# kjedrzejewski/video-cycle_gan-upscaling

Measured on AMD Instinct MI355X. Metric: upscaled frames/s (train step, G+D fwd+bwd) at 256->512, higher is better.
Workload: dtype f32; 1 GPU; C2: make_upscaler_orig((512,512,3),k=3,x2,res=9) + PatchGAN-70, batch 8/GPU, gan2 wiring, Wasserstein + pixel-MSE, faithful 3-call step incl. predict pass; global_batch=8, frame=256x256->512x512, parallelism=dp1, launch=hipGraph replay

## Files before the change

### video-cycle_gan-upscaling_amd/build.py

```python
import glob
import os
import subprocess
import sys
from concurrent.futures import ThreadPoolExecutor

HERE = os.path.dirname(os.path.abspath(__file__))
ROOT = os.path.dirname(HERE)
CSRC = os.path.join(HERE, "csrc")
OUT = os.path.join(HERE, "libvcg_hip.so")
SOURCES = ["conv_fwd.hip", "conv_rowchain.hip", "conv_transpose.hip", "conv_wgrad.hip", "norm.hip", "elementwise.hip", "dense.hip", "bf16_layout.hip", "bf16_conv3x3_3ch.hip", "bf16_convt3x3.hip", "bf16_conv9x9_to3.hip", "bf16_norm.hip", "bf16_wgrad.hip", "bf16_wgrad9.hip", "bf16_gconv.hip", "bf16_gwgrad.hip", "bf16_head.hip", "bf16_wgrad3.hip", "bf16_attn.hip", "bf16_incep.hip", "bf16_vgg.hip", "api.hip"]
FLAGS = ["-O3", "--offload-arch=gfx950", "-fPIC", "-std=c++17", "-I", os.path.join(ROOT, "include"), "-I", CSRC,
         "-Wno-unused-value", "-Wno-c++20-extensions"]


def _hipcc():
    for c in (os.environ.get("HIPCC"), "/opt/rocm/bin/hipcc", "hipcc"):
        if c and (os.path.isabs(c) and os.path.exists(c) or not os.path.isabs(c)):
            return c
    raise RuntimeError("hipcc not found")


def _stale(target, deps):
    if not os.path.exists(target):
        return True
    t = os.path.getmtime(target)
    return any(os.path.getmtime(d) > t for d in deps)


def build(force=False, verbose=True, extra_flags=(), objdir=None, out=OUT, jobs=4):
    hipcc = _hipcc()
    objdir = objdir or os.path.join(HERE, "build")
    flags = FLAGS + list(extra_flags)
    hdrs = sorted(glob.glob(os.path.join(CSRC, "*.hpp"))) + [os.path.join(ROOT, "include", "vcg.h")]
    objs, cmds = [], []
    os.makedirs(objdir, exist_ok=True)
    for s in SOURCES:
        src = os.path.join(CSRC, s)
        obj = os.path.join(objdir, s.replace(".hip", ".o"))
        objs.append(obj)
        if force or _stale(obj, [src] + hdrs):
            cmds.append([hipcc, "-c", src, "-o", obj] + flags)

    def run(cmd):
        if verbose:
            print(" ".join(cmd), flush=True)
        subprocess.run(cmd, check=True)

    with ThreadPoolExecutor(max_workers=jobs) as ex:
        list(ex.map(run, cmds))
    if force or cmds or _stale(out, objs):
        run([hipcc, "-shared", "-fPIC", "--offload-arch=gfx950", "-o", out] + objs)
    return out


if __name__ == "__main__":
    print(build(force="--force" in sys.argv))
```

### video-cycle_gan-upscaling_amd/csrc/api.hip

```cpp
#include "vcg_common.hpp"

int vcg_internal_conv(const float* x, const float* w, float* y, int n, int cin, int h, int wd, int cout, int oh,
                      int ow, int kh, int kw, int stride, int pad_top, int pad_left, int flip, const vcg_epilogue* ep,
                      int smallm, int ws_t, int ws_m, int ws_k, hipStream_t st, float* stats = nullptr, const float* scale = nullptr,
                      const float* shift = nullptr);
int vcg_internal_convt(const float* x, const float* w, float* y, int n, int cin, int h, int wd, int cout, int oh,
                       int ow, int k, int cby, int cbx, const vcg_epilogue* ep, hipStream_t st);
size_t vcg_internal_wgrad_ws(int n, int mtot, int ah, int aw, int jctot, int kh, int kw, int S);
int vcg_internal_wgrad(const float* A, const float* B, float* dw, float* db, int n, int mtot, int ah, int aw,
                       int jctot, int bh, int bw, int kh, int kw, int S, int pt, int pl_, int flip, int ts, int sm,
                       int sj, void* ws, size_t ws_bytes, hipStream_t st);

namespace {

int check_desc(const vcg_conv_desc* d) {
    if (d == nullptr) return VCG_E_NULL;
    if (d->n <= 0 || d->cin <= 0 || d->h <= 0 || d->w <= 0 || d->cout <= 0 || d->oh <= 0 || d->ow <= 0)
        return VCG_E_SHAPE;
    if (d->kh <= 0 || d->kw <= 0 || d->stride < 1 || d->stride > 3) return VCG_E_UNSUPPORTED;
    if (d->pad_top < 0 || d->pad_left < 0 || d->pad_top >= d->kh || d->pad_left >= d->kw) return VCG_E_SHAPE;
    return VCG_OK;
}

inline bool use_smallm(int mch, int kh, int kw, int stride) { return stride == 1 && kh == kw && kh >= 3 && mch * kw <= 32; }

}

extern "C" {

const char* vcg_version(void) { return "vcg-hip 0.1 (gfx950, fp32 MFMA 32x32x2)"; }

const char* vcg_error_string(int code) {
    switch (code) {
        case VCG_OK: return "ok";
        case VCG_E_NULL: return "required pointer is NULL";
        case VCG_E_SHAPE: return "inconsistent or unsupported dimensions";
        case VCG_E_UNSUPPORTED: return "kernel size / stride / padding combination not instantiated";
        case VCG_E_WORKSPACE: return "workspace missing or too small";
        default: return code > 0 ? hipGetErrorString((hipError_t)code) : "unknown error";
    }
}

int vcg_conv2d_fwd(const vcg_conv_desc* d, const float* x, const float* w_hwio, float* y, const vcg_epilogue* ep,
                   vcg_stream_t stream) {
    int rc = check_desc(d);
    if (rc) return rc;
    VCG_CHECK_PTR(x); VCG_CHECK_PTR(w_hwio); VCG_CHECK_PTR(y);
    if ((d->oh - 1) * d->stride - d->pad_top >= d->h || (d->ow - 1) * d->stride - d->pad_left >= d->w) return VCG_E_SHAPE;
    const bool sm = use_smallm(d->cout, d->kh, d->kw, d->stride);
    return vcg_internal_conv(x, w_hwio, y, d->n, d->cin, d->h, d->w, d->cout, d->oh, d->ow, d->kh, d->kw, d->stride,
                             d->pad_top, d->pad_left, 0, ep, sm ? 1 : 0, d->cin * d->cout, 1, d->cout,
                             (hipStream_t)stream);
}

static bool conv_stats_tiles(const vcg_conv_desc* d, int* tiles_per_image) {
    const bool k3 = d->kh == 3 && d->kw == 3, k4 = d->kh == 4 && d->kw == 4;
    if (!(k3 || k4) || d->stride > 2 || d->cin <= 3) return false;
    const bool sm = use_smallm(d->cout, d->kh, d->kw, d->stride);
    if (sm) return false;
    const int xt = (k3 && d->stride == 1 && d->ow > 32) ? 2 : 1;
    *tiles_per_image = ceil_div(d->ow, 32 * xt) * ceil_div(d->oh, 8);
    return true;
}

int vcg_conv2d_stats_records(const vcg_conv_desc* d, int stats_mode) {
    int rc = check_desc(d);
    if (rc) return rc;
    int tpi = 0;
    if (!conv_stats_tiles(d, &tpi) || (stats_mode != VCG_STATS_BATCH && stats_mode != VCG_STATS_INSTANCE)) return VCG_E_UNSUPPORTED;
    const long all = (long)tpi * d->n;
    if (all > 0x3fffffffL) return VCG_E_UNSUPPORTED;
    return (int)(stats_mode == VCG_STATS_INSTANCE ? tpi : all);
}

int vcg_conv2d_fwd_stats(const vcg_conv_desc* d, const float* x, const float* w_hwio, const float* bias, float* y, float* stats,
                         vcg_stream_t stream) {
    int rc = check_desc(d);
    if (rc) return rc;
    VCG_CHECK_PTR(x); VCG_CHECK_PTR(w_hwio); VCG_CHECK_PTR(y); VCG_CHECK_PTR(stats);
    if ((d->oh - 1) * d->stride - d->pad_top >= d->h || (d->ow - 1) * d->stride - d->pad_left >= d->w) return VCG_E_SHAPE;
    int tpi = 0;
    if (!conv_stats_tiles(d, &tpi)) return VCG_E_UNSUPPORTED;
    vcg_epilogue ep{};
    ep.bias = bias;
    ep.act = VCG_ACT_NONE;
    return vcg_internal_conv(x, w_hwio, y, d->n, d->cin, d->h, d->w, d->cout, d->oh, d->ow, d->kh, d->kw, d->stride, d->pad_top, d->pad_left, 0,
                             &ep, 0, d->cin * d->cout, 1, d->cout, (hipStream_t)stream, stats);
}

int vcg_conv2d_fwd_affine(const vcg_conv_desc* d, const float* x, const float* w_hwio, float* y, const vcg_epilogue* ep, const float* scale,
                          const float* shift, vcg_stream_t stream) {
    int rc = check_desc(d);
    if (rc) return rc;
    VCG_CHECK_PTR(x); VCG_CHECK_PTR(w_hwio); VCG_CHECK_PTR(y); VCG_CHECK_PTR(scale); VCG_CHECK_PTR(shift);
    if ((d->oh - 1) * d->stride - d->pad_top >= d->h || (d->ow - 1) * d->stride - d->pad_left >= d->w) return VCG_E_SHAPE;
    if (use_smallm(d->cout, d->kh, d->kw, d->stride)) return VCG_E_UNSUPPORTED;
    return vcg_internal_conv(x, w_hwio, y, d->n, d->cin, d->h, d->w, d->cout, d->oh, d->ow, d->kh, d->kw, d->stride, d->pad_top, d->pad_left, 0,
                             ep, 0, d->cin * d->cout, 1, d->cout, (hipStream_t)stream, nullptr, scale, shift);
}

int vcg_conv2d_dgrad(const vcg_conv_desc* d, const float* dy, const float* w_hwio, const float* w_hwoi, float* dx,
                     const float* residual, vcg_stream_t stream) {
    int rc = check_desc(d);
    if (rc) return rc;
    VCG_CHECK_PTR(dy); VCG_CHECK_PTR(dx);
    vcg_epilogue ep{};
    ep.residual = residual;
    hipStream_t st = (hipStream_t)stream;
    if (d->stride == 1) {
        const int pt = d->kh - 1 - d->pad_top, pl = d->kw - 1 - d->pad_left;
        if (use_smallm(d->cin, d->kh, d->kw, 1)) {
            VCG_CHECK_PTR(w_hwio);
            return vcg_internal_conv(dy, w_hwio, dx, d->n, d->cout, d->oh, d->ow, d->cin, d->h, d->w, d->kh, d->kw, 1,
                                     pt, pl, 1, &ep, 1, d->cin * d->cout, d->cout, 1, st);
        }
        VCG_CHECK_PTR(w_hwoi);
        return vcg_internal_conv(dy, w_hwoi, dx, d->n, d->cout, d->oh, d->ow, d->cin, d->h, d->w, d->kh, d->kw, 1, pt,
                                 pl, 1, &ep, 0, 0, 0, 0, st);
    }
    if (d->kh != d->kw || d->stride != 2) return VCG_E_UNSUPPORTED;
    VCG_CHECK_PTR(w_hwoi);
    return vcg_internal_convt(dy, w_hwoi, dx, d->n, d->cout, d->oh, d->ow, d->cin, d->h, d->w, d->kh, d->pad_top,
                              d->pad_left, &ep, st);
}

size_t vcg_conv2d_wgrad_workspace_bytes(const vcg_conv_desc* d) {
    if (check_desc(d)) return 0;
    size_t a;
    if (d->stride == 1 && d->cout <= 3)
        a = vcg_internal_wgrad_ws(d->n, d->cin, d->h, d->w, d->cout, d->kh, d->kw, 1);
    else
        a = vcg_internal_wgrad_ws(d->n, d->cout, d->oh, d->ow, d->cin, d->kh, d->kw, d->stride);
    const size_t b = vcg_channel_sum_workspace_bytes(d->n, d->cout, d->oh * d->ow);
    return a > b ? a : b;
}

int vcg_conv2d_wgrad(const vcg_conv_desc* d, const float* x, const float* dy, float* dw_hwio, float* dbias, void* ws,
                     size_t ws_bytes, vcg_stream_t stream) {
    int rc = check_desc(d);
    if (rc) return rc;
    VCG_CHECK_PTR(x); VCG_CHECK_PTR(dy); VCG_CHECK_PTR(dw_hwio);
    hipStream_t st = (hipStream_t)stream;
    const int cc = d->cin * d->cout;
    if (d->stride == 1 && d->cout <= 3) {
        rc = vcg_internal_wgrad(x, dy, dw_hwio, nullptr, d->n, d->cin, d->h, d->w, d->cout, d->oh, d->ow, d->kh, d->kw,
                                1, d->kh - 1 - d->pad_top, d->kw - 1 - d->pad_left, 1, cc, d->cout, 1, ws, ws_bytes, st);
    } else {
        rc = vcg_internal_wgrad(dy, x, dw_hwio, dbias, d->n, d->cout, d->oh, d->ow, d->cin, d->h, d->w, d->kh, d->kw,
                                d->stride, d->pad_top, d->pad_left, 0, cc, 1, d->cout, ws, ws_bytes, st);
        dbias = nullptr;
    }
    if (rc) return rc;
    if (dbias) {
        if (ws_bytes < vcg_channel_sum_workspace_bytes(d->n, d->cout, d->oh * d->ow)) return VCG_E_WORKSPACE;
        rc = vcg_channel_sum(dy, d->n, d->cout, d->oh * d->ow, dbias, ws, ws_bytes, stream);
    }
    return rc;
}

int vcg_conv_transpose2d_fwd(const vcg_conv_desc* d, const float* x, const float* w_hwio_t, float* y,
                             const vcg_epilogue* ep, vcg_stream_t stream) {
    int rc = check_desc(d);
    if (rc) return rc;
    VCG_CHECK_PTR(x); VCG_CHECK_PTR(w_hwio_t); VCG_CHECK_PTR(y);
    if (d->stride != 2 || d->kh != d->kw) return VCG_E_UNSUPPORTED;
    if (d->oh > 2 * d->h || d->ow > 2 * d->w) return VCG_E_SHAPE;
    return vcg_internal_convt(x, w_hwio_t, y, d->n, d->cin, d->h, d->w, d->cout, d->oh, d->ow, d->kh, d->pad_top,
                              d->pad_left, ep, (hipStream_t)stream);
}

int vcg_conv_transpose2d_dgrad(const vcg_conv_desc* d, const float* dy, const float* w_hwoi, float* dx,
                               const float* residual, vcg_stream_t stream) {
    int rc = check_desc(d);
    if (rc) return rc;
    VCG_CHECK_PTR(dy); VCG_CHECK_PTR(w_hwoi); VCG_CHECK_PTR(dx);
    if (d->stride != 2) return VCG_E_UNSUPPORTED;
    vcg_epilogue ep{};
    ep.residual = residual;
    return vcg_internal_conv(dy, w_hwoi, dx, d->n, d->cout, d->oh, d->ow, d->cin, d->h, d->w, d->kh, d->kw, 2,
                             d->pad_top, d->pad_left, 0, &ep, 0, 0, 0, 0, (hipStream_t)stream);
}

size_t vcg_conv_transpose2d_wgrad_workspace_bytes(const vcg_conv_desc* d) {
    if (check_desc(d)) return 0;
    size_t a = vcg_internal_wgrad_ws(d->n, d->cin, d->h, d->w, d->cout, d->kh, d->kw, 2);
    size_t b = vcg_channel_sum_workspace_bytes(d->n, d->cout, d->oh * d->ow);
    return a > b ? a : b;
}

int vcg_conv_transpose2d_wgrad(const vcg_conv_desc* d, const float* x, const float* dy, float* dw_hwoi, float* dbias,
                               void* ws, size_t ws_bytes, vcg_stream_t stream) {
    int rc = check_desc(d);
    if (rc) return rc;
    VCG_CHECK_PTR(x); VCG_CHECK_PTR(dy); VCG_CHECK_PTR(dw_hwoi);
    if (d->stride != 2) return VCG_E_UNSUPPORTED;
    rc = vcg_internal_wgrad(x, dy, dw_hwoi, nullptr, d->n, d->cin, d->h, d->w, d->cout, d->oh, d->ow, d->kh, d->kw, 2,
                            d->pad_top, d->pad_left, 0, d->cin * d->cout, 1, d->cin, ws, ws_bytes, (hipStream_t)stream);
    if (rc) return rc;
    if (dbias) {
        if (ws_bytes < vcg_channel_sum_workspace_bytes(d->n, d->cout, d->oh * d->ow)) return VCG_E_WORKSPACE;
        rc = vcg_channel_sum(dy, d->n, d->cout, d->oh * d->ow, dbias, ws, ws_bytes, stream);
    }
    return rc;
}
// ... 3 lines not shown
```

### video-cycle_gan-upscaling_amd/csrc/conv_fwd.hip

```cpp
#include "vcg_common.hpp"
#include <type_traits>

namespace {

struct ConvParams {
    const float* x;
    const float* w;
    float* y;
    const float* bias;
    const float* prelu;
    const float* residual;
    int n, cin, h, w_, cout, oh, ow, pad_top, pad_left;
    int tiles_x, tiles_y, co_blocks;
    int act;
    float alpha;
    int flip;
    int ws_t, ws_m, ws_k;
    float* stats;
    const float* scale;
    const float* shift;
};

template <int KH, int KW, int S, int CK, int XT>
struct ConvCfg {
// ... 495 lines not shown
            const int ch = ci0 + ci;
            const bool ok = e < C::W_ELEMS && ch < p.cin && mi < mrows;
            const int mch = mi / KW, kx = mi % KW;
            int tap = ky * KW + kx;
            if (p.flip) tap = KH * KW - 1 - tap;
            rw[i] = buf_load(rwt, ok ? 4u * (unsigned)(tap * p.ws_t + mch * p.ws_m + ch * p.ws_k) : VCG_OOB);
        }
    };
    auto store_chunk = [&]() {
#pragma unroll
        for (int i = 0; i < C::IN_PT; ++i) {
            const int e = tid + i * 256;
            if (e < C::IN_ELEMS) s_in[e] = rin[i];
        }
#pragma unroll
        for (int i = 0; i < C::W_PT; ++i) {
            const int e = tid + i * 256;
            if (e < C::W_ELEMS) s_w[e] = rw[i];
        }
    };

    f32x16 acc[2][2];
#pragma unroll
    for (int i = 0; i < 2; ++i)
#pragma unroll
        for (int j = 0; j < 2; ++j)
#pragma unroll
            for (int r = 0; r < 16; ++r) acc[i][j][r] = 0.f;

    const float* bbase = s_in + half * C::PLANE + (wv * 2) * C::XW + l31;
    const float* abase = s_w + half * KH * 32 + l31;

    const int nchunks = (p.cin + CK - 1) / CK;
    load_chunk(0);
    for (int c = 0; c < nchunks; ++c) {
        __syncthreads();
        store_chunk();
        __syncthreads();
        if (c + 1 < nchunks) load_chunk((c + 1) * CK);
#pragma unroll
        for (int cp = 0; cp < CK / 2; ++cp) {
#pragma unroll
            for (int ky = 0; ky < KH; ++ky) {
                const float a = abase[(cp * 2 * KH + ky) * 32];
                const float b00 = bbase[cp * 2 * C::PLANE + ky * C::XW];
                const float b01 = bbase[cp * 2 * C::PLANE + ky * C::XW + 32];
                const float b10 = bbase[cp * 2 * C::PLANE + (ky + 1) * C::XW];
                const float b11 = bbase[cp * 2 * C::PLANE + (ky + 1) * C::XW + 32];
                acc[0][0] = mfma32(a, b00, acc[0][0]);
                acc[0][1] = mfma32(a, b01, acc[0][1]);
                acc[1][0] = mfma32(a, b10, acc[1][0]);
                acc[1][1] = mfma32(a, b11, acc[1][1]);
            }
        }
    }

    float* s_p = smem + wv * 32 * C::PST;
#pragma unroll
    for (int rt = 0; rt < 2; ++rt) {
        __syncthreads();
#pragma unroll
        for (int xt = 0; xt < 2; ++xt)
#pragma unroll
            for (int r = 0; r < 16; ++r) s_p[mfma_row(r, lane) * C::PST + xt * 32 + l31] = acc[rt][xt][r];
        __syncthreads();
        const int oy = oy0 + wv * 2 + rt;
        const int ox = ox0 + lane;
        if (lane < C::OUTW && oy < p.oh && ox < p.ow) {
            for (int mch = 0; mch < p.cout; ++mch) {
                float v = 0.f;
#pragma unroll
                for (int kx = 0; kx < KW; ++kx) v += s_p[(mch * KW + kx) * C::PST + lane + kx];
                const float bv = p.bias ? p.bias[mch] : 0.f;
                const float al = (p.act == VCG_ACT_PRELU) ? p.prelu[mch] : p.alpha;
                const size_t idx = (((size_t)n * p.cout + mch) * p.oh + oy) * p.ow + ox;
                v = apply_act(v + bv, p.act, al);
                if (p.residual) v += p.residual[idx];
                p.y[idx] = v;
            }
        }
    }
}

template <int K>
__global__ __launch_bounds__(256) void conv_cout1_kernel(const ConvParams p) {
    __shared__ float red[4][64];
    const int tid = threadIdx.x, xl = tid & 63;
    const int cg = __builtin_amdgcn_readfirstlane(tid >> 6);
    int b = blockIdx.x;
    const int seg = b % p.tiles_x; b /= p.tiles_x;
    const int oy = b % p.oh;
    const int n = b / p.oh;
    const int ox = seg * 64 + xl, gx0 = ox - p.pad_left, gy0 = oy - p.pad_top;
    const int hw = p.h * p.w_;
    const vcg_rsrc rx = make_rsrc(p.x + (size_t)n * p.cin * hw, (size_t)p.cin * hw * sizeof(float));
    unsigned coff[K];
#pragma unroll
    for (int kx = 0; kx < K; ++kx) coff[kx] = (unsigned)(gx0 + kx) < (unsigned)p.w_ ? 4u * (unsigned)(gx0 + kx) : VCG_OOB;
    float acc = 0.f;
#pragma unroll 1
    for (int c = cg; c < p.cin; c += 4) {
        float wr[K * K];
#pragma unroll
        for (int t = 0; t < K * K; ++t) wr[t] = p.w[(p.flip ? K * K - 1 - t : t) * p.ws_t + c * p.ws_k];
#pragma unroll
        for (int ky = 0; ky < K; ++ky) {
            const int gy = gy0 + ky;
            const bool rok = (unsigned)gy < (unsigned)p.h;
            const unsigned rbase = 4u * (unsigned)(c * hw + gy * p.w_);
#pragma unroll
            for (int kx = 0; kx < K; ++kx) acc += buf_load(rx, rok && coff[kx] != VCG_OOB ? rbase + coff[kx] : VCG_OOB) * wr[ky * K + kx];
        }
    }
    red[cg][xl] = acc;
    __syncthreads();
    if (cg == 0 && ox < p.ow) {
        float v = ((red[0][xl] + red[1][xl]) + (red[2][xl] + red[3][xl])) + (p.bias ? p.bias[0] : 0.f);
        if (p.act == VCG_ACT_LRELU) v = v >= 0.f ? v : v * p.alpha;
        else if (p.act == VCG_ACT_TANH) v = tanhf(v);
        const size_t o = ((size_t)n * p.oh + oy) * p.ow + ox;
        if (p.residual) v += p.residual[o];
        p.y[o] = v;
    }
}

template <int K>
int launch_cout1(ConvParams p, hipStream_t st) {
    p.tiles_x = ceil_div(p.ow, 64);
    const long grid = (long)p.tiles_x * p.oh * p.n;
    if (grid <= 0 || grid > 0x7fffffffL) return VCG_E_SHAPE;
    hipLaunchKernelGGL(conv_cout1_kernel<K>, dim3((unsigned)grid), dim3(256), 0, st, p);
    VCG_LAUNCH_CHECK();
    return VCG_OK;
}

template <typename Kern>
int launch_with_lds(Kern kern, int grid, size_t lds, const ConvParams& p, hipStream_t st) {
    if (int e = vcg_allow_dyn_lds(reinterpret_cast<const void*>(kern), lds)) return e;
    hipLaunchKernelGGL(kern, dim3(grid), dim3(256), lds, st, p);
    VCG_LAUNCH_CHECK();
    return VCG_OK;
}

bool conv_block_fits(int oh, int ow, int ck, int h, int w) {
    const unsigned long long lim = 0xFFFFFFE0ull;
    return 64ull * oh * ow * sizeof(float) < lim && (unsigned long long)ck * h * w * sizeof(float) < lim;
}

template <int KH, int KW, int S, int CK, int XT>
int launch_conv(ConvParams p, hipStream_t st) {
    using C = ConvCfg<KH, KW, S, CK, XT>;
    if (!conv_block_fits(p.oh, p.ow, CK, p.h, p.w_)) return VCG_E_UNSUPPORTED;
    p.tiles_x = ceil_div(p.ow, 32 * XT);
    p.tiles_y = ceil_div(p.oh, C::ROWS);
    p.co_blocks = ceil_div(p.cout, 64);
    const long grid = (long)p.tiles_x * p.tiles_y * p.co_blocks * p.n;
    if (grid <= 0 || grid > 0x7fffffffL) return VCG_E_SHAPE;
    if (p.stats && p.scale) return VCG_E_UNSUPPORTED;
    if (p.stats) {
        if constexpr ((KH == 3 && KW == 3 && S <= 2) || (KH == 4 && KW == 4 && S <= 2))
            return launch_with_lds(conv_fwd_kernel<KH, KW, S, CK, XT, true>, (int)grid, C::LDS_BYTES, p, st);
        else
            return VCG_E_UNSUPPORTED;
    }
    if (p.scale) {
        if constexpr (S == 1 && ((KH == 3 && KW == 3) || (KH == 5 && KW == 5)))
            return launch_with_lds(conv_fwd_kernel<KH, KW, S, CK, XT, false, true>, (int)grid, C::LDS_BYTES, p, st);
        else
            return VCG_E_UNSUPPORTED;
    }
    return launch_with_lds(conv_fwd_kernel<KH, KW, S, CK, XT>, (int)grid, C::LDS_BYTES, p, st);
}

int device_cu_count() {
    static const int cus = [] {
        int dev = 0, v = 0;
        if (hipGetDevice(&dev) != hipSuccess || hipDeviceGetAttribute(&v, hipDeviceAttributeMultiprocessorCount, dev) != hipSuccess) return 0;
        return v;
    }();
    return cus;
}

template <int KH, int KW, int S>
int launch_c3(ConvParams p, hipStream_t st) {
    using C = C3Cfg<KH, KW, S>;
    if (!conv_block_fits(p.oh, p.ow, 3, p.h, p.w_)) return VCG_E_UNSUPPORTED;
    p.tiles_x = ceil_div(p.ow, 32);
    p.tiles_y = ceil_div(p.oh, C::ROWS);
    p.co_blocks = ceil_div(p.cout, 64);
    const long tiles = (long)p.tiles_x * p.tiles_y * p.co_blocks * p.n;
    if (tiles <= 0 || tiles > 0x7fffffffL) return VCG_E_SHAPE;
    const int cus = device_cu_count();
    if (cus <= 0) return VCG_E_UNSUPPORTED;
    long grid = tiles < 2L * cus ? tiles : 2L * cus;
    grid -= grid % p.co_blocks;
    if (grid < p.co_blocks) grid = p.co_blocks;
    return launch_with_lds(conv_c3_kernel<KH, KW, S>, (int)grid, C::LDS_BYTES, p, st);
}

template <int KH, int KW, int CK>
int launch_smallm(ConvParams p, hipStream_t st) {
    using C = SmallCfg<KH, KW, CK>;
    p.tiles_x = ceil_div(p.ow, C::OUTW);
    p.tiles_y = ceil_div(p.oh, C::ROWS);
    p.co_blocks = 1;
    const long grid = (long)p.tiles_x * p.tiles_y * p.n;
    if (grid <= 0 || grid > 0x7fffffffL) return VCG_E_SHAPE;
    return launch_with_lds(conv_smallm_kernel<KH, KW, CK>, (int)grid, C::LDS_BYTES, p, st);
}

}

int vcg_internal_conv9_rowchain(const float* x, const float* w, float* y, int n, int cin, int h, int wd, int cout, const float* bias, int act,
                                int ws_t, int ws_m, int ws_k, hipStream_t st);

int vcg_internal_conv(const float* x, const float* w, float* y, int n, int cin, int h, int wd, int cout,
                      int oh, int ow, int kh, int kw, int stride, int pad_top, int pad_left, int flip,
                      const vcg_epilogue* ep, int smallm, int ws_t, int ws_m, int ws_k, hipStream_t st, float* stats, const float* scale, const float* shift) {
    ConvParams p{};
    p.x = x; p.w = w; p.y = y; p.stats = stats;
    if (stats && (smallm || cin <= 3)) return VCG_E_UNSUPPORTED;
    if (scale && (smallm || stats || cin <= 3)) return VCG_E_UNSUPPORTED;
    if (scale && shift == nullptr) return VCG_E_NULL;
    p.scale = scale; p.shift = scale ? shift : nullptr;
    p.bias = ep ? ep->bias : nullptr;
    p.prelu = ep ? ep->prelu_alpha : nullptr;
    p.residual = ep ? ep->residual : nullptr;
    p.act = ep ? ep->act : VCG_ACT_NONE;
    p.alpha = ep ? ep->act_alpha : 0.f;
    if (p.act == VCG_ACT_PRELU && p.prelu == nullptr) return VCG_E_NULL;
    p.n = n; p.cin = cin; p.h = h; p.w_ = wd; p.cout = cout; p.oh = oh; p.ow = ow;
    p.pad_top = pad_top; p.pad_left = pad_left; p.flip = flip;
    p.ws_t = ws_t; p.ws_m = ws_m; p.ws_k = ws_k;
    if (n <= 0 || cin <= 0 || cout <= 0 || oh <= 0 || ow <= 0) return VCG_E_SHAPE;
    if (smallm) {
        if (stride != 1 || cout * kw > 32) return VCG_E_UNSUPPORTED;
        if (kh == 9 && kw == 9 && !flip && pad_top == 4 && pad_left == 4 && oh == h && ow == wd && !p.prelu && !p.residual) {
            const int rc = vcg_internal_conv9_rowchain(x, w, y, n, cin, h, wd, cout, p.bias, p.act, ws_t, ws_m, ws_k, st);
            if (rc != VCG_E_UNSUPPORTED) return rc;
        }
        if (cout == 1 && cin >= 64 && kh == kw && ws_m == 1 && !p.prelu && (size_t)cin * h * wd * 4 <= 0xFFFFFFE0u) {
            if (kh == 3) return launch_cout1<3>(p, st);
            if (kh == 4) return launch_cout1<4>(p, st);
            if (kh == 5) return launch_cout1<5>(p, st);
        }
        if (kh == 9 && kw == 9) return launch_smallm<9, 9, 8>(p, st);
        if (kh == 4 && kw == 4) return launch_smallm<4, 4, 8>(p, st);
        if (kh == 3 && kw == 3) return launch_smallm<3, 3, 8>(p, st);
        if (kh == 5 && kw == 5) return launch_smallm<5, 5, 8>(p, st);
        return VCG_E_UNSUPPORTED;
    }
    if (p.act == VCG_ACT_TANH) return VCG_E_UNSUPPORTED;
    if (cin <= 3) {
        if (kh == 9 && kw == 9 && stride == 1) return launch_c3<9, 9, 1>(p, st);
        if (kh == 3 && kw == 3 && stride == 1) return launch_c3<3, 3, 1>(p, st);
        if (kh == 4 && kw == 4 && stride == 2) return launch_c3<4, 4, 2>(p, st);
        if (kh == 5 && kw == 5 && stride == 1) return launch_c3<5, 5, 1>(p, st);
    }
    const bool wide = ow > 32;
    if (kh == 3 && kw == 3 && stride == 1) return wide ? launch_conv<3, 3, 1, 8, 2>(p, st) : launch_conv<3, 3, 1, 8, 1>(p, st);
    if (kh == 5 && kw == 5 && stride == 1) return launch_conv<5, 5, 1, 8, 1>(p, st);
    if (scale) return VCG_E_UNSUPPORTED;
    if (kh == 3 && kw == 3 && stride == 2) return launch_conv<3, 3, 2, 8, 1>(p, st);
    if (kh == 4 && kw == 4 && stride == 1) return launch_conv<4, 4, 1, 8, 1>(p, st);
    if (kh == 4 && kw == 4 && stride == 2) return launch_conv<4, 4, 2, 4, 1>(p, st);
    if (kh == 5 && kw == 5 && stride == 2) return launch_conv<5, 5, 2, 4, 1>(p, st);
    if (kh == 5 && kw == 5 && stride == 3) return launch_conv<5, 5, 3, 4, 1>(p, st);
    if (kh == 9 && kw == 9 && stride == 1) return launch_conv<9, 9, 1, 4, 1>(p, st);
    if (stride == 1) {
        if (kh == 1 && kw == 1) return launch_conv<1, 1, 1, 8, 1>(p, st);
        if (kh == 1 && kw == 3) return launch_conv<1, 3, 1, 8, 1>(p, st);
        if (kh == 3 && kw == 1) return launch_conv<3, 1, 1, 8, 1>(p, st);
        if (kh == 1 && kw == 5) return launch_conv<1, 5, 1, 8, 1>(p, st);
        if (kh == 5 && kw == 1) return launch_conv<5, 1, 1, 8, 1>(p, st);
        if (kh == 1 && kw == 7) return launch_conv<1, 7, 1, 8, 1>(p, st);
        if (kh == 7 && kw == 1) return launch_conv<7, 1, 1, 8, 1>(p, st);
    }
    return VCG_E_UNSUPPORTED;
}
```

### video-cycle_gan-upscaling_amd/csrc/conv_transpose.hip

```cpp
#include "vcg_common.hpp"
#include <type_traits>

namespace {

struct ConvTParams {
    const float* x;
    const float* w;
    float* y;
    const float* bias;
    const float* prelu;
    const float* residual;
    int n, cin, h, w_, cout, oh, ow;
    int tiles_x, tiles_y, co_blocks;
    int act;
    float alpha;
};

constexpr int phase_of(int k, int cb) { return (((k - cb) % 2) + 2) % 2; }
constexpr int d_of(int k, int cb) { return (k - cb - phase_of(k, cb)) / 2; }
constexpr int dmin_of(int K, int cb) { int m = 1000; for (int k = 0; k < K; ++k) m = d_of(k, cb) < m ? d_of(k, cb) : m; return m; }
constexpr int dmax_of(int K, int cb) { int m = -1000; for (int k = 0; k < K; ++k) m = d_of(k, cb) > m ? d_of(k, cb) : m; return m; }

template <int K, int CBY, int CBX, int CK, int MT>
struct ConvTCfg {
// ... 125 lines not shown
        }
    }

    const int qy = qy0 + wv, qx = qx0 + l31;
    const bool vec_ok = (p.ow % 2) == 0;
    const bool full = vec_ok && (co0 + C::MB <= p.cout) && (2 * (qy0 + C::QROWS) <= p.oh) && (2 * (qx0 + 32) <= p.ow);
    const int plane = p.oh * p.ow;
    const size_t img = (size_t)n * p.cout * plane;
    float* yimg = p.y + img;
    const float* rimg = p.residual ? p.residual + img : nullptr;
    const int ob = (co0 + 4 * half) * plane + (2 * qy) * p.ow + 2 * qx;
    const float* bp = p.bias ? p.bias : vcg_zero_word;
    const int bmask = p.bias ? ~0 : 0;
    const bool is_prelu = p.act == VCG_ACT_PRELU;
    const float* ap = is_prelu ? p.prelu : vcg_zero_word;
    const int amask = is_prelu ? ~0 : 0;
    const float slope_u = (p.act == VCG_ACT_LRELU) ? p.alpha : 1.f;
    auto emit = [&](auto guard_tag, auto res_tag) {
        constexpr bool GUARD = decltype(guard_tag)::value, RES = decltype(res_tag)::value;
#pragma unroll
        for (int mt = 0; mt < MT; ++mt) {
#pragma unroll
            for (int r = 0; r < 16; ++r) {
                const int row = mt * 32 + mfma_row(r, lane);
                const int co = co0 + row;
                const bool co_ok = !GUARD || co < p.cout;
                const int cs = co_ok ? co : co0;
                const float bvv = bp[cs & bmask];
                const float pa = ap[cs & amask];
                const float al = is_prelu ? pa : slope_u;
#pragma unroll
                for (int py = 0; py < 2; ++py) {
                    const int o = ob + (row - 4 * half) * plane + py * p.ow;
                    float v0 = acc[py][0][mt][r] + bvv, v1 = acc[py][1][mt][r] + bvv;
                    v0 = v0 >= 0.f ? v0 : v0 * al;
                    v1 = v1 >= 0.f ? v1 : v1 * al;
                    if (!GUARD) {
                        if (RES) { const float2 rr = *reinterpret_cast<const float2*>(rimg + o); v0 += rr.x; v1 += rr.y; }
                        *reinterpret_cast<float2*>(yimg + o) = make_float2(v0, v1);
                    } else {
                        const int oy = 2 * qy + py, ox = 2 * qx;
                        if (co_ok && oy < p.oh && ox < p.ow) {
                            if (vec_ok) {
                                if (RES) { const float2 rr = *reinterpret_cast<const float2*>(rimg + o); v0 += rr.x; v1 += rr.y; }
                                *reinterpret_cast<float2*>(yimg + o) = make_float2(v0, v1);
                            } else {
                                if (RES) v0 += rimg[o];
                                yimg[o] = v0;
                                if (ox + 1 < p.ow) {
                                    if (RES) v1 += rimg[o + 1];
                                    yimg[o + 1] = v1;
                                }
                            }
                        }
                    }
                }
            }
        }
    };
    using T_ = std::true_type;
    using F_ = std::false_type;
    if (full) {
        if (p.residual) emit(F_{}, T_{}); else emit(F_{}, F_{});
    } else {
        if (p.residual) emit(T_{}, T_{}); else emit(T_{}, F_{});
    }
}

template <int K, int CBY, int CBX, int CK, int MT>
int launch_convt(ConvTParams p, hipStream_t st) {
    using C = ConvTCfg<K, CBY, CBX, CK, MT>;
    p.tiles_x = ceil_div(ceil_div(p.ow, 2), 32);
    p.tiles_y = ceil_div(ceil_div(p.oh, 2), C::QROWS);
    p.co_blocks = ceil_div(p.cout, C::MB);
    const long grid = (long)p.tiles_x * p.tiles_y * p.co_blocks * p.n;
    if (grid <= 0 || grid > 0x7fffffffL) return VCG_E_SHAPE;
    auto kern = convt_kernel<K, CBY, CBX, CK, MT>;
    if (int e = vcg_allow_dyn_lds(reinterpret_cast<const void*>(kern), C::LDS_BYTES)) return e;
    hipLaunchKernelGGL(kern, dim3((int)grid), dim3(256), C::LDS_BYTES, st, p);
    VCG_LAUNCH_CHECK();
    return VCG_OK;
}

}

int vcg_internal_convt(const float* x, const float* w, float* y, int n, int cin, int h, int wd, int cout,
                       int oh, int ow, int k, int cby, int cbx, const vcg_epilogue* ep, hipStream_t st) {
    ConvTParams p{};
    p.x = x; p.w = w; p.y = y;
    p.bias = ep ? ep->bias : nullptr;
    p.prelu = ep ? ep->prelu_alpha : nullptr;
    p.residual = ep ? ep->residual : nullptr;
    p.act = ep ? ep->act : VCG_ACT_NONE;
    p.alpha = ep ? ep->act_alpha : 0.f;
    if (p.act == VCG_ACT_PRELU && p.prelu == nullptr) return VCG_E_NULL;
    if (p.act == VCG_ACT_TANH) return VCG_E_UNSUPPORTED;
    p.n = n; p.cin = cin; p.h = h; p.w_ = wd; p.cout = cout; p.oh = oh; p.ow = ow;
    if (n <= 0 || cin <= 0 || cout <= 0 || oh <= 0 || ow <= 0) return VCG_E_SHAPE;
#define VCG_CT(K_, A_, B_, CK_, MT_) if (k == K_ && cby == A_ && cbx == B_) return launch_convt<K_, A_, B_, CK_, MT_>(p, st)
    VCG_CT(3, 0, 0, 16, 1); VCG_CT(3, 0, 1, 16, 1); VCG_CT(3, 1, 0, 16, 1); VCG_CT(3, 1, 1, 16, 1);
    VCG_CT(4, 1, 1, 16, 1);
    VCG_CT(5, 1, 1, 8, 2); VCG_CT(5, 1, 2, 8, 2); VCG_CT(5, 2, 1, 8, 2); VCG_CT(5, 2, 2, 8, 2);
#undef VCG_CT
    return VCG_E_UNSUPPORTED;
}
```

Measured before the change: 138.7 frames/s.

## Add specialized kernels for cout=1 head fwd/dgrad and small-cout stride-2 dgrad

Moves the cout=1 forward kernel into a new file and widens it to 16 channel groups per block. Weights are loaded once per wave and broadcast with readlane, and the input loads are double-buffered. Adds a dedicated cout=1 dgrad kernel that computes the 3x3 to 5x5 gradient taps once per pixel and scatters them over channel blocks, replacing the generic conv path. Adds a small-output transposed-conv kernel for stride-2 dgrad into 3 or fewer channels (the PatchGAN first layer), with weights staged in LDS and packed FMAs. These target the PatchGAN head and first-layer backward, which map poorly onto the general kernels. The cost is more specialized code paths and larger blocks, which may lower occupancy.

```diff
diff --git a/video-cycle_gan-upscaling_amd/build.py b/video-cycle_gan-upscaling_amd/build.py
--- a/video-cycle_gan-upscaling_amd/build.py
+++ b/video-cycle_gan-upscaling_amd/build.py
@@ -8,7 +8,7 @@
 ROOT = os.path.dirname(HERE)
 CSRC = os.path.join(HERE, "csrc")
 OUT = os.path.join(HERE, "libvcg_hip.so")
-SOURCES = ["conv_fwd.hip", "conv_rowchain.hip", "conv_transpose.hip", "conv_wgrad.hip", "norm.hip", "elementwise.hip", "dense.hip", "bf16_layout.hip", "bf16_conv3x3_3ch.hip", "bf16_convt3x3.hip", "bf16_conv9x9_to3.hip", "bf16_norm.hip", "bf16_wgrad.hip", "bf16_wgrad9.hip", "bf16_gconv.hip", "bf16_gwgrad.hip", "bf16_head.hip", "bf16_wgrad3.hip", "bf16_attn.hip", "bf16_incep.hip", "bf16_vgg.hip", "api.hip"]
+SOURCES = ["conv_fwd.hip", "conv_head.hip", "conv_rowchain.hip", "conv_transpose.hip", "conv_wgrad.hip", "norm.hip", "elementwise.hip", "dense.hip", "bf16_layout.hip", "bf16_conv3x3_3ch.hip", "bf16_convt3x3.hip", "bf16_conv9x9_to3.hip", "bf16_norm.hip", "bf16_wgrad.hip", "bf16_wgrad9.hip", "bf16_gconv.hip", "bf16_gwgrad.hip", "bf16_head.hip", "bf16_wgrad3.hip", "bf16_attn.hip", "bf16_incep.hip", "bf16_vgg.hip", "api.hip"]
 FLAGS = ["-O3", "--offload-arch=gfx950", "-fPIC", "-std=c++17", "-I", os.path.join(ROOT, "include"), "-I", CSRC,
          "-Wno-unused-value", "-Wno-c++20-extensions"]
 
diff --git a/video-cycle_gan-upscaling_amd/csrc/api.hip b/video-cycle_gan-upscaling_amd/csrc/api.hip
--- a/video-cycle_gan-upscaling_amd/csrc/api.hip
+++ b/video-cycle_gan-upscaling_amd/csrc/api.hip
@@ -6,6 +6,10 @@
                       const float* shift = nullptr);
 int vcg_internal_convt(const float* x, const float* w, float* y, int n, int cin, int h, int wd, int cout, int oh,
                        int ow, int k, int cby, int cbx, const vcg_epilogue* ep, hipStream_t st);
+int vcg_internal_convt_small(const float* x, const float* w, float* y, int n, int cin, int h, int wd, int cout, int oh, int ow, int k,
+                             int cby, int cbx, const float* residual, hipStream_t st);
+int vcg_internal_cout1_dgrad(const float* dy, const float* w, float* dx, int n, int cin, int h, int wd, int oh, int ow, int k, int pad_top,
+                             int pad_left, const float* residual, hipStream_t st);
 size_t vcg_internal_wgrad_ws(int n, int mtot, int ah, int aw, int jctot, int kh, int kw, int S);
 int vcg_internal_wgrad(const float* A, const float* B, float* dw, float* db, int n, int mtot, int ah, int aw,
                        int jctot, int bh, int bw, int kh, int kw, int S, int pt, int pl_, int flip, int ts, int sm,
@@ -115,11 +119,20 @@
                                      pt, pl, 1, &ep, 1, d->cin * d->cout, d->cout, 1, st);
         }
         VCG_CHECK_PTR(w_hwoi);
+        if (d->cout == 1 && d->cin >= 64 && d->kh == d->kw && d->kh >= 3 && d->kh <= 5) {
+            rc = vcg_internal_cout1_dgrad(dy, w_hwoi, dx, d->n, d->cin, d->h, d->w, d->oh, d->ow, d->kh, d->pad_top, d->pad_left, residual, st);
+            if (rc != VCG_E_UNSUPPORTED) return rc;
+        }
         return vcg_internal_conv(dy, w_hwoi, dx, d->n, d->cout, d->oh, d->ow, d->cin, d->h, d->w, d->kh, d->kw, 1, pt,
                                  pl, 1, &ep, 0, 0, 0, 0, st);
     }
     if (d->kh != d->kw || d->stride != 2) return VCG_E_UNSUPPORTED;
     VCG_CHECK_PTR(w_hwoi);
+    if (d->cin <= 3 && (d->kh == 3 || d->kh == 4)) {
+        rc = vcg_internal_convt_small(dy, w_hwoi, dx, d->n, d->cout, d->oh, d->ow, d->cin, d->h, d->w, d->kh, d->pad_top, d->pad_left,
+                                      residual, st);
+        if (rc != VCG_E_UNSUPPORTED) return rc;
+    }
     return vcg_internal_convt(dy, w_hwoi, dx, d->n, d->cout, d->oh, d->ow, d->cin, d->h, d->w, d->kh, d->pad_top,
                               d->pad_left, &ep, st);
 }
diff --git a/video-cycle_gan-upscaling_amd/csrc/conv_fwd.hip b/video-cycle_gan-upscaling_amd/csrc/conv_fwd.hip
--- a/video-cycle_gan-upscaling_amd/csrc/conv_fwd.hip
+++ b/video-cycle_gan-upscaling_amd/csrc/conv_fwd.hip
@@ -601,58 +601,6 @@
     }
 }
 
-template <int K>
-__global__ __launch_bounds__(256) void conv_cout1_kernel(const ConvParams p) {
-    __shared__ float red[4][64];
-    const int tid = threadIdx.x, xl = tid & 63;
-    const int cg = __builtin_amdgcn_readfirstlane(tid >> 6);
-    int b = blockIdx.x;
-    const int seg = b % p.tiles_x; b /= p.tiles_x;
-    const int oy = b % p.oh;
-    const int n = b / p.oh;
-    const int ox = seg * 64 + xl, gx0 = ox - p.pad_left, gy0 = oy - p.pad_top;
-    const int hw = p.h * p.w_;
-    const vcg_rsrc rx = make_rsrc(p.x + (size_t)n * p.cin * hw, (size_t)p.cin * hw * sizeof(float));
-    unsigned coff[K];
-#pragma unroll
-    for (int kx = 0; kx < K; ++kx) coff[kx] = (unsigned)(gx0 + kx) < (unsigned)p.w_ ? 4u * (unsigned)(gx0 + kx) : VCG_OOB;
-    float acc = 0.f;
-#pragma unroll 1
-    for (int c = cg; c < p.cin; c += 4) {
-        float wr[K * K];
-#pragma unroll
-        for (int t = 0; t < K * K; ++t) wr[t] = p.w[(p.flip ? K * K - 1 - t : t) * p.ws_t + c * p.ws_k];
-#pragma unroll
-        for (int ky = 0; ky < K; ++ky) {
-            const int gy = gy0 + ky;
-            const bool rok = (unsigned)gy < (unsigned)p.h;
-            const unsigned rbase = 4u * (unsigned)(c * hw + gy * p.w_);
-#pragma unroll
-            for (int kx = 0; kx < K; ++kx) acc += buf_load(rx, rok && coff[kx] != VCG_OOB ? rbase + coff[kx] : VCG_OOB) * wr[ky * K + kx];
-        }
-    }
-    red[cg][xl] = acc;
-    __syncthreads();
-    if (cg == 0 && ox < p.ow) {
-        float v = ((red[0][xl] + red[1][xl]) + (red[2][xl] + red[3][xl])) + (p.bias ? p.bias[0] : 0.f);
-        if (p.act == VCG_ACT_LRELU) v = v >= 0.f ? v : v * p.alpha;
-        else if (p.act == VCG_ACT_TANH) v = tanhf(v);
-        const size_t o = ((size_t)n * p.oh + oy) * p.ow + ox;
-        if (p.residual) v += p.residual[o];
-        p.y[o] = v;
-    }
-}
-
-template <int K>
-int launch_cout1(ConvParams p, hipStream_t st) {
-    p.tiles_x = ceil_div(p.ow, 64);
-    const long grid = (long)p.tiles_x * p.oh * p.n;
-    if (grid <= 0 || grid > 0x7fffffffL) return VCG_E_SHAPE;
-    hipLaunchKernelGGL(conv_cout1_kernel<K>, dim3((unsigned)grid), dim3(256), 0, st, p);
-    VCG_LAUNCH_CHECK();
-    return VCG_OK;
-}
-
 template <typename Kern>
 int launch_with_lds(Kern kern, int grid, size_t lds, const ConvParams& p, hipStream_t st) {
     if (int e = vcg_allow_dyn_lds(reinterpret_cast<const void*>(kern), lds)) return e;
@@ -732,6 +680,10 @@
 
 int vcg_internal_conv9_rowchain(const float* x, const float* w, float* y, int n, int cin, int h, int wd, int cout, const float* bias, int act,
                                 int ws_t, int ws_m, int ws_k, hipStream_t st);
+
+int vcg_internal_cout1_fwd(const float* x, const float* w, float* y, int n, int cin, int h, int wd, int oh, int ow, int k, int pad_top,
+                           int pad_left, int flip, int ws_t, int ws_k, const float* bias, int act, float alpha, const float* residual,
+                           hipStream_t st);
 
 int vcg_internal_conv(const float* x, const float* w, float* y, int n, int cin, int h, int wd, int cout,
                       int oh, int ow, int kh, int kw, int stride, int pad_top, int pad_left, int flip,
@@ -758,10 +710,10 @@
             const int rc = vcg_internal_conv9_rowchain(x, w, y, n, cin, h, wd, cout, p.bias, p.act, ws_t, ws_m, ws_k, st);
             if (rc != VCG_E_UNSUPPORTED) return rc;
         }
-        if (cout == 1 && cin >= 64 && kh == kw && ws_m == 1 && !p.prelu && (size_t)cin * h * wd * 4 <= 0xFFFFFFE0u) {
-            if (kh == 3) return launch_cout1<3>(p, st);
-            if (kh == 4) return launch_cout1<4>(p, st);
-            if (kh == 5) return launch_cout1<5>(p, st);
+        if (cout == 1 && cin >= 64 && kh == kw && ws_m == 1 && !p.prelu) {
+            const int rc = vcg_internal_cout1_fwd(x, w, y, n, cin, h, wd, oh, ow, kh, pad_top, pad_left, flip, ws_t, ws_k, p.bias, p.act, p.alpha,
+                                                  p.residual, st);
+            if (rc != VCG_E_UNSUPPORTED) return rc;
         }
         if (kh == 9 && kw == 9) return launch_smallm<9, 9, 8>(p, st);
         if (kh == 4 && kw == 4) return launch_smallm<4, 4, 8>(p, st);
diff --git a/video-cycle_gan-upscaling_amd/csrc/conv_head.hip b/video-cycle_gan-upscaling_amd/csrc/conv_head.hip
--- /dev/null
+++ b/video-cycle_gan-upscaling_amd/csrc/conv_head.hip
@@ -0,0 +1,190 @@
+#include "vcg_common.hpp"
+
+namespace {
+
+struct HeadParams {
+    const float* x;
+    const float* w;
+    float* y;
+    const float* bias;
+    const float* residual;
+    int n, cin, h, w_, oh, ow, pad_top, pad_left, flip, ws_t, ws_k, act;
+    float alpha;
+    int tiles_x, cblocks;
+};
+
+constexpr int FWD_CG = 16;
+
+template <int K>
+__global__ __launch_bounds__(64 * FWD_CG) void conv_cout1_kernel(const HeadParams p) {
+    __shared__ float red[FWD_CG][64];
+    const int tid = threadIdx.x, xl = tid & 63;
+    const int cg = __builtin_amdgcn_readfirstlane(tid >> 6);
+    int b = blockIdx.x;
+    const int seg = b % p.tiles_x; b /= p.tiles_x;
+    const int oy = b % p.oh;
+    const int n = b / p.oh;
+    const int ox = seg * 64 + xl, gx0 = ox - p.pad_left, gy0 = oy - p.pad_top;
+    const int hw = p.h * p.w_;
+    const vcg_rsrc rx = make_rsrc(p.x + (size_t)n * p.cin * hw, (size_t)p.cin * hw * sizeof(float));
+    unsigned off[K * K];
+#pragma unroll
+    for (int ky = 0; ky < K; ++ky)
+#pragma unroll
+        for (int kx = 0; kx < K; ++kx) {
+            const int gy = gy0 + ky, gx = gx0 + kx;
+            off[ky * K + kx] = ((unsigned)gy < (unsigned)p.h && (unsigned)gx < (unsigned)p.w_) ? 4u * (unsigned)(gy * p.w_ + gx) : VCG_OOB;
+        }
+    auto load_plane = [&](float (&v)[K * K], int c) {
+        const int so = (int)((unsigned)c * (unsigned)hw * 4u);
+#pragma unroll
+        for (int t = 0; t < K * K; ++t) v[t] = __builtin_bit_cast(float, __builtin_amdgcn_raw_buffer_load_b32(rx, (int)off[t], so, 0));
+    };
+    constexpr int KK = K * K, WR = (KK + 1) / 2;
+    const vcg_rsrc rw = make_rsrc(p.w, ((size_t)(KK - 1) * p.ws_t + (size_t)(p.cin - 1) * p.ws_k + 1) * sizeof(float));
+    float acc = 0.f;
+    const int ni = cg < p.cin ? (p.cin - cg + FWD_CG - 1) / FWD_CG : 0;
+    for (int i0 = 0; i0 < ni; i0 += 32) {
+        float wl[WR];
+#pragma unroll
+        for (int j = 0; j < WR; ++j) {
+            const int t = 2 * j + (xl >> 5), i = i0 + (xl & 31);
+            const int tap = p.flip ? KK - 1 - t : t;
+            wl[j] = buf_load(rw, (t < KK && i < ni) ? 4u * (unsigned)(tap * p.ws_t + (cg + FWD_CG * i) * p.ws_k) : VCG_OOB);
+        }
+        auto fma_plane = [&](const float (&v)[KK], int il) {
+#pragma unroll
+            for (int t = 0; t < KK; ++t)
+                acc = fmaf(v[t], __builtin_bit_cast(float, __builtin_amdgcn_readlane(__builtin_bit_cast(int, wl[t >> 1]), il + 32 * (t & 1))), acc);
+        };
+        const int i1 = i0 + 32 < ni ? i0 + 32 : ni;
+        float va[KK], vb[KK];
+        load_plane(va, cg + FWD_CG * i0);
+        int i = i0;
+#pragma unroll 1
+        for (; i + 1 < i1; i += 2) {
+            load_plane(vb, cg + FWD_CG * (i + 1));
+            __builtin_amdgcn_sched_barrier(0);
+            fma_plane(va, i - i0);
+            __builtin_amdgcn_sched_barrier(0);
+            load_plane(va, cg + FWD_CG * (i + 2 < i1 ? i + 2 : i + 1));
+            __builtin_amdgcn_sched_barrier(0);
+            fma_plane(vb, i + 1 - i0);
+            __builtin_amdgcn_sched_barrier(0);
+        }
+        if (i < i1) fma_plane(va, i - i0);
+    }
+    red[cg][xl] = acc;
+    __syncthreads();
+    if (cg == 0 && ox < p.ow) {
+        float s[FWD_CG / 4];
+#pragma unroll
+        for (int i = 0; i < FWD_CG / 4; ++i) s[i] = (red[4 * i][xl] + red[4 * i + 1][xl]) + (red[4 * i + 2][xl] + red[4 * i + 3][xl]);
+        float v = ((s[0] + s[1]) + (s[2] + s[3])) + (p.bias ? p.bias[0] : 0.f);
+        if (p.act == VCG_ACT_LRELU) v = v >= 0.f ? v : v * p.alpha;
+        else if (p.act == VCG_ACT_TANH) v = tanhf(v);
+        const size_t o = ((size_t)n * p.oh + oy) * p.ow + ox;
+        if (p.residual) v += p.residual[o];
+        p.y[o] = v;
+    }
+}
+
+template <int K>
+int launch_cout1(HeadParams p, hipStream_t st) {
+    p.tiles_x = ceil_div(p.ow, 64);
+    const long grid = (long)p.tiles_x * p.oh * p.n;
+    if (grid <= 0 || grid > 0x7fffffffL) return VCG_E_SHAPE;
+    hipLaunchKernelGGL(conv_cout1_kernel<K>, dim3((unsigned)grid), dim3(64 * FWD_CG), 0, st, p);
+    VCG_LAUNCH_CHECK();
+    return VCG_OK;
+}
+
+constexpr int DG_CPW = 32;
+
+template <int K>
+__global__ __launch_bounds__(256) void cout1_dgrad_kernel(const HeadParams p) {
+    const int tid = threadIdx.x, xl = tid & 63;
+    const int wv = __builtin_amdgcn_readfirstlane(tid >> 6);
+    int b = blockIdx.x;
+    const int seg = b % p.tiles_x; b /= p.tiles_x;
+    const int cb = b % p.cblocks;  b /= p.cblocks;
+    const int iy = b % p.h;
+    const int n = b / p.h;
+    const int ix = seg * 64 + xl;
+    const int hw = p.h * p.w_, plane = p.oh * p.ow;
+    const vcg_rsrc rg = make_rsrc(p.x + (size_t)n * plane, (size_t)plane * sizeof(float));
+    float g[K * K];
+#pragma unroll
+    for (int ky = 0; ky < K; ++ky)
+#pragma unroll
+        for (int kx = 0; kx < K; ++kx) {
+            const int gy = iy + p.pad_top - ky, gx = ix + p.pad_left - kx;
+            g[ky * K + kx] = buf_load(rg, ((unsigned)gy < (unsigned)p.oh && (unsigned)gx < (unsigned)p.ow) ? 4u * (unsigned)(gy * p.ow + gx) : VCG_OOB);
+        }
+    const size_t img = (size_t)n * p.cin * hw;
+    const vcg_rsrc ry = make_rsrc(p.y + img, (size_t)p.cin * hw * sizeof(float));
+    const vcg_rsrc rr = make_rsrc(p.residual ? p.residual + img : vcg_zero_word, p.residual ? (size_t)p.cin * hw * sizeof(float) : 0);
+    const bool has_res = p.residual != nullptr;
+    const unsigned voff = ix < p.w_ ? 4u * (unsigned)(iy * p.w_ + ix) : VCG_OOB;
+    const int c0 = (cb * 4 + wv) * DG_CPW;
+    const int c1 = c0 + DG_CPW < p.cin ? c0 + DG_CPW : p.cin;
+    constexpr int WR = (K * K + 1) / 2;
+    const vcg_rsrc rw = make_rsrc(p.w, (size_t)K * K * p.cin * sizeof(float));
+    float wl[WR];
+#pragma unroll
+    for (int j = 0; j < WR; ++j) {
+        const int t = 2 * j + (xl >> 5), c = c0 + (xl & 31);
+        wl[j] = buf_load(rw, (t < K * K && c < p.cin) ? 4u * (unsigned)(t * p.cin + c) : VCG_OOB);
+    }
+    for (int c = c0; c < c1; ++c) {
+        const int cl = c - c0;
+        float v = 0.f;
+#pragma unroll
+        for (int t = 0; t < K * K; ++t)
+            v = fmaf(g[t], __builtin_bit_cast(float, __builtin_amdgcn_readlane(__builtin_bit_cast(int, wl[t >> 1]), cl + 32 * (t & 1))), v);
+        const int so = (int)((unsigned)c * (unsigned)hw * 4u);
+        if (has_res) v += __builtin_bit_cast(float, __builtin_amdgcn_raw_buffer_load_b32(rr, (int)voff, so, 0));
+        __builtin_amdgcn_raw_buffer_store_b32(__builtin_bit_cast(unsigned, v), ry, (int)voff, so, 0);
+    }
+}
+
+template <int K>
+int launch_cout1_dgrad(HeadParams p, hipStream_t st) {
+    p.tiles_x = ceil_div(p.w_, 64);
+    p.cblocks = ceil_div(p.cin, 4 * DG_CPW);
+    const long grid = (long)p.tiles_x * p.cblocks * p.h * p.n;
+    if (grid <= 0 || grid > 0x7fffffffL) return VCG_E_SHAPE;
+    hipLaunchKernelGGL(cout1_dgrad_kernel<K>, dim3((unsigned)grid), dim3(256), 0, st, p);
+    VCG_LAUNCH_CHECK();
+    return VCG_OK;
+}
+
+}
+
+int vcg_internal_cout1_fwd(const float* x, const float* w, float* y, int n, int cin, int h, int wd, int oh, int ow, int k, int pad_top,
+                           int pad_left, int flip, int ws_t, int ws_k, const float* bias, int act, float alpha, const float* residual,
+                           hipStream_t st) {
+    if ((unsigned long long)cin * h * wd * sizeof(float) > 0xFFFFFFE0ull) return VCG_E_UNSUPPORTED;
+    HeadParams p{};
+    p.x = x; p.w = w; p.y = y; p.bias = bias; p.residual = residual;
+    p.n = n; p.cin = cin; p.h = h; p.w_ = wd; p.oh = oh; p.ow = ow; p.pad_top = pad_top; p.pad_left = pad_left;
+    p.flip = flip; p.ws_t = ws_t; p.ws_k = ws_k; p.act = act; p.alpha = alpha;
+    if (k == 3) return launch_cout1<3>(p, st);
+    if (k == 4) return launch_cout1<4>(p, st);
+    if (k == 5) return launch_cout1<5>(p, st);
+    return VCG_E_UNSUPPORTED;
+}
+
+int vcg_internal_cout1_dgrad(const float* dy, const float* w, float* dx, int n, int cin, int h, int wd, int oh, int ow, int k, int pad_top,
+                             int pad_left, const float* residual, hipStream_t st) {
+    if (n <= 0 || cin <= 0 || h <= 0 || wd <= 0 || oh <= 0 || ow <= 0) return VCG_E_UNSUPPORTED;
+    if ((unsigned long long)cin * h * wd * sizeof(float) >= 0xFFFFFFE0ull || (unsigned long long)oh * ow * sizeof(float) >= 0xFFFFFFE0ull)
+        return VCG_E_UNSUPPORTED;
+    HeadParams p{};
+    p.x = dy; p.w = w; p.y = dx; p.residual = residual;
+    p.n = n; p.cin = cin; p.h = h; p.w_ = wd; p.oh = oh; p.ow = ow; p.pad_top = pad_top; p.pad_left = pad_left;
+    if (k == 3) return launch_cout1_dgrad<3>(p, st);
+    if (k == 4) return launch_cout1_dgrad<4>(p, st);
+    if (k == 5) return launch_cout1_dgrad<5>(p, st);
+    return VCG_E_UNSUPPORTED;
+}
diff --git a/video-cycle_gan-upscaling_amd/csrc/conv_transpose.hip b/video-cycle_gan-upscaling_amd/csrc/conv_transpose.hip
--- a/video-cycle_gan-upscaling_amd/csrc/conv_transpose.hip
+++ b/video-cycle_gan-upscaling_amd/csrc/conv_transpose.hip
@@ -231,6 +231,147 @@
     return VCG_OK;
 }
 
+typedef float f32x2 __attribute__((ext_vector_type(2)));
+
+template <int K, int CBY, int CBX>
+struct ConvTSmallCfg {
+    static constexpr int SQY = 2;
+    static constexpr int ROWS = 4 * SQY;
+    static constexpr int DMINY = dmin_of(K, CBY), DMAXY = dmax_of(K, CBY);
+    static constexpr int DMINX = dmin_of(K, CBX), DMAXX = dmax_of(K, CBX);
+    static constexpr int NRY = SQY + DMAXY - DMINY, NCX = 1 + DMAXX - DMINX;
+    static constexpr int T = K * K;
+    static constexpr int WS4 = T;
+};
+
+template <int K, int CBY, int CBX>
+__global__ __launch_bounds__(256, 3) void convt_small_kernel(const ConvTParams p) {
+    using C = ConvTSmallCfg<K, CBY, CBX>;
+    extern __shared__ __attribute__((aligned(16))) float smem[];
+    const int tid = threadIdx.x, lane = tid & 63;
+    const int wv = __builtin_amdgcn_readfirstlane(tid >> 6);
+    for (int e = tid; e < p.cin * C::WS4 * 4; e += 256) {
+        const int c = e / (C::WS4 * 4), r = e % (C::WS4 * 4);
+        const int t = r / 4, m = r % 4;
+        smem[e] = (t < C::T && m < p.cout) ? p.w[((size_t)t * p.cin + c) * p.cout + m] : 0.f;
+    }
+    __syncthreads();
+
+    int b = blockIdx.x;
+    const int tx = b % p.tiles_x; b /= p.tiles_x;
+    const int ty = b % p.tiles_y;
+    const int n = b / p.tiles_y;
+    const int qx = tx * 64 + lane, qy0 = (ty * 4 + wv) * C::SQY;
+    const int hw = p.h * p.w_;
+    const vcg_rsrc rx = make_rsrc(p.x + (size_t)n * p.cin * hw, (size_t)p.cin * hw * sizeof(float));
+    unsigned off[C::NRY][C::NCX];
+#pragma unroll
+    for (int r = 0; r < C::NRY; ++r)
+#pragma unroll
+        for (int c = 0; c < C::NCX; ++c) {
+            const int gy = qy0 + r - C::DMAXY, gx = qx + c - C::DMAXX;
+            off[r][c] = ((unsigned)gy < (unsigned)p.h && (unsigned)gx < (unsigned)p.w_) ? 4u * (unsigned)(gy * p.w_ + gx) : VCG_OOB;
+        }
+    auto load_plane = [&](float (&v)[C::NRY][C::NCX], int ci) {
+        const int so = (int)((unsigned)ci * (unsigned)hw * 4u);
+#pragma unroll
+        for (int r = 0; r < C::NRY; ++r)
+#pragma unroll
+            for (int c = 0; c < C::NCX; ++c)
+                v[r][c] = __builtin_bit_cast(float, __builtin_amdgcn_raw_buffer_load_b32(rx, (int)off[r][c], so, 0));
+    };
+
+    f32x2 acc[C::SQY][2][2][2];
+#pragma unroll
+    for (int i = 0; i < C::SQY * 8; ++i) (&acc[0][0][0][0])[i] = f32x2{0.f, 0.f};
+
+    const f32x4* s_w4 = reinterpret_cast<const f32x4*>(smem);
+    auto fma_plane = [&](const float (&cur)[C::NRY][C::NCX], int ci) {
+        f32x4 wr[C::T];
+#pragma unroll
+        for (int i = 0; i < C::T; ++i) wr[i] = s_w4[ci * C::WS4 + i];
+#pragma unroll
+        for (int ky = 0; ky < K; ++ky)
+#pragma unroll
+            for (int kx = 0; kx < K; ++kx) {
+                const int t = ky * K + kx;
+                const int py = phase_of(ky, CBY), px = phase_of(kx, CBX);
+                const int ry = C::DMAXY - d_of(ky, CBY), cx = C::DMAXX - d_of(kx, CBX);
+#pragma unroll
+                for (int r = 0; r < C::SQY; ++r) {
+                    const f32x2 in2 = {cur[r + ry][cx], cur[r + ry][cx]};
+                    acc[r][py][px][0] = __builtin_elementwise_fma(f32x2{wr[t].x, wr[t].y}, in2, acc[r][py][px][0]);
+                    acc[r][py][px][1] = __builtin_elementwise_fma(f32x2{wr[t].z, wr[t].w}, in2, acc[r][py][px][1]);
+                }
+            }
+    };
+    float va[C::NRY][C::NCX], vb[C::NRY][C::NCX];
+    load_plane(va, 0);
+    int ci = 0;
+#pragma unroll 1
+    for (; ci + 1 < p.cin; ci += 2) {
+        load_plane(vb, ci + 1);
+        __builtin_amdgcn_sched_barrier(0);
+        fma_plane(va, ci);
+        __builtin_amdgcn_sched_barrier(0);
+        load_plane(va, ci + 2 < p.cin ? ci + 2 : p.cin - 1);
+        __builtin_amdgcn_sched_barrier(0);
+        fma_plane(vb, ci + 1);
+        __builtin_amdgcn_sched_barrier(0);
+    }
+    if (ci < p.cin) fma_plane(va, ci);
+
+    const int plane = p.oh * p.ow;
+    const size_t img = (size_t)n * p.cout * plane;
+    float* yimg = p.y + img;
+    const float* rimg = p.residual ? p.residual + img : nullptr;
+    const bool vec_ok = (p.ow % 2) == 0;
+    const int ox = 2 * qx;
+    if (ox >= p.ow) return;
+#pragma unroll
+    for (int r = 0; r < C::SQY; ++r)
+#pragma unroll
+        for (int py = 0; py < 2; ++py) {
+            const int oy = 2 * (qy0 + r) + py;
+            if (oy >= p.oh) continue;
+#pragma unroll
+            for (int m = 0; m < 3; ++m) {
+                if (m >= p.cout) continue;
+                const size_t o = (size_t)m * plane + (size_t)oy * p.ow + ox;
+                float v0 = acc[r][py][0][m >> 1][m & 1], v1 = acc[r][py][1][m >> 1][m & 1];
+                if (vec_ok) {
+                    if (rimg) { const float2 rr = *reinterpret_cast<const float2*>(rimg + o); v0 += rr.x; v1 += rr.y; }
+                    *reinterpret_cast<float2*>(yimg + o) = make_float2(v0, v1);
+                } else {
+                    if (rimg) v0 += rimg[o];
+                    yimg[o] = v0;
+                    if (ox + 1 < p.ow) {
+                        if (rimg) v1 += rimg[o + 1];
+                        yimg[o + 1] = v1;
+                    }
+                }
+            }
+        }
+}
+
+template <int K>
+bool convt_small_fits(const ConvTParams& p) {
+    const size_t lds = (size_t)p.cin * (K * K) * 16;
+    return lds <= 64 * 1024 && (unsigned long long)p.cin * p.h * p.w_ * sizeof(float) < 0xFFFFFFE0ull;
+}
+
+template <int K, int CBY, int CBX>
+int launch_convt_small(ConvTParams p, hipStream_t st) {
+    using C = ConvTSmallCfg<K, CBY, CBX>;
+    p.tiles_x = ceil_div(ceil_div(p.ow, 2), 64);
+    p.tiles_y = ceil_div(ceil_div(p.oh, 2), C::ROWS);
+    const long grid = (long)p.tiles_x * p.tiles_y * p.n;
+    if (grid <= 0 || grid > 0x7fffffffL) return VCG_E_SHAPE;
+    hipLaunchKernelGGL((convt_small_kernel<K, CBY, CBX>), dim3((int)grid), dim3(256), (size_t)p.cin * C::WS4 * 16, st, p);
+    VCG_LAUNCH_CHECK();
+    return VCG_OK;
+}
+
 }
 
 int vcg_internal_convt(const float* x, const float* w, float* y, int n, int cin, int h, int wd, int cout,
@@ -253,3 +394,17 @@
 #undef VCG_CT
     return VCG_E_UNSUPPORTED;
 }
+
+int vcg_internal_convt_small(const float* x, const float* w, float* y, int n, int cin, int h, int wd, int cout, int oh, int ow, int k,
+                             int cby, int cbx, const float* residual, hipStream_t st) {
+    if (n <= 0 || cin <= 0 || cout <= 0 || cout > 3 || h <= 0 || wd <= 0 || oh <= 0 || ow <= 0) return VCG_E_UNSUPPORTED;
+    ConvTParams p{};
+    p.x = x; p.w = w; p.y = y; p.residual = residual;
+    p.act = VCG_ACT_NONE;
+    p.n = n; p.cin = cin; p.h = h; p.w_ = wd; p.cout = cout; p.oh = oh; p.ow = ow;
+#define VCG_CTS(K_, A_, B_) if (k == K_ && cby == A_ && cbx == B_ && convt_small_fits<K_>(p)) return launch_convt_small<K_, A_, B_>(p, st)
+    VCG_CTS(3, 0, 0); VCG_CTS(3, 0, 1); VCG_CTS(3, 1, 0); VCG_CTS(3, 1, 1);
+    VCG_CTS(4, 1, 1);
+#undef VCG_CTS
+    return VCG_E_UNSUPPORTED;
+}
```

Measured after the change: 139.5 frames/s (median of 6 runs). No clear change (+0.6%).
